# ShangtongZhang/DeepRL

Hardware: NVIDIA H100
Metric: gradient-updates/sec (DQN batch 512, 84x84x4 synthetic) (higher is better)
Workload: dtype bf16

## Files before the change

deeprl_b200/csrc/gemm.cu:

```cuda
#include <cuda.h>
#include <cstdlib>
#include "common.cuh"
#include "wgmma.cuh"

namespace b2rl {

constexpr int GEMM_BM = 128;
constexpr int GEMM_BK = 64;
constexpr int GEMM_THREADS = 384;
constexpr int MMA_WARPS = 8;

__device__ __forceinline__ uint32_t s2u(const void* p) { return (uint32_t)__cvta_generic_to_shared(p); }

__device__ __forceinline__ void mb_init(uint64_t* bar, uint32_t count) {
  asm volatile("mbarrier.init.shared::cta.b64 [%0], %1;" ::"r"(s2u(bar)), "r"(count));
}
__device__ __forceinline__ void mb_expect_tx(uint64_t* bar, uint32_t bytes) {
  asm volatile("mbarrier.arrive.expect_tx.shared::cta.b64 _, [%0], %1;" ::"r"(s2u(bar)), "r"(bytes) : "memory");
}
__device__ __forceinline__ void mb_arrive(uint64_t* bar) {
  asm volatile("mbarrier.arrive.shared::cta.b64 _, [%0];" ::"r"(s2u(bar)) : "memory");
}
__device__ __forceinline__ void mb_wait(uint64_t* bar, uint32_t parity) {
  asm volatile(
// ... 655 lines not shown
__device__ __forceinline__ uint32_t lds32(uint32_t addr) {
  uint32_t v;
  asm volatile("ld.shared.u32 %0, [%1];" : "=r"(v) : "r"(addr));
  return v;
}
__device__ __forceinline__ void sts128(uint32_t addr, const int4 v) {
  asm volatile("st.shared.v4.b32 [%0], {%1, %2, %3, %4};" ::"r"(addr), "r"(v.x), "r"(v.y), "r"(v.z), "r"(v.w) : "memory");
}

__device__ __forceinline__ uint32_t slab_chunk(uint32_t slab, uint32_t slab_b, int rl, int j) {
  return j < 8 ? slab + (uint32_t)(rl * 128 + ((j ^ (rl & 7)) << 4)) : slab_b + (uint32_t)(rl * 32 + (((j - 8) ^ ((rl >> 2) & 1)) << 4));
}

template <int J0, int NJ>
__device__ __forceinline__ void u8_store_chunks(uint32_t stage, uint32_t slab, uint32_t slab_b, int rl, int so, int fstride,
                                                int frame_w) {
  uint32_t w0[NJ], w1[NJ];
#pragma unroll
  for (int jj = 0; jj < NJ; ++jj) {
    const int j = J0 + jj;
    w0[jj] = w1[jj] = 0;
    if (so >= 0) {
      const uint32_t src = stage + (uint32_t)((j >> 1) * fstride + so + (2 * (j & 1)) * frame_w);
      w0[jj] = lds32(src);
      w1[jj] = lds32(src + frame_w);
    }
  }
#pragma unroll
  for (int jj = 0; jj < NJ; ++jj) sts128(slab_chunk(slab, slab_b, rl, J0 + jj), cvt8_u8_bf16(w0[jj], w1[jj]));
}

template <int NT, int NCH>
__device__ __forceinline__ void u8_convert(const U8Src& u, const uint8_t* stage_p, uint8_t* slab_p, uint8_t* slab_b_p, int R0,
                                           int slab_rows, int slots, int tid, int bar_id) {
  const uint32_t stage = s2u(stage_p), slab = s2u(slab_p), slab_b = NCH > 8 ? s2u(slab_b_p) : 0u;
  const int rowb = 4 * u.frame_w, fstride = slots * rowb;
  const int q0 = R0 / u.G;
  const int qb1 = (q0 / u.G + 1) * u.G;
  const int seg1 = (u.nf * fstride + 127) & ~127;
  const int rl0 = tid & 127;
  if (rl0 < slab_rows) {
    const int r = R0 + rl0;
    int so = -1;
    if (r < u.rows) {
      const int q = r / u.G;
      so = (q >= qb1 ? seg1 + (q - qb1) * rowb : (q - q0) * rowb) + 4 * (r - q * u.G);
    }
    if (NT == 128) {
      u8_store_chunks<0, NCH>(stage, slab, slab_b, rl0, so, fstride, u.frame_w);
    } else if (tid < 128) {
      u8_store_chunks<0, NCH / 2>(stage, slab, slab_b, rl0, so, fstride, u.frame_w);
    } else {
      u8_store_chunks<NCH / 2, NCH / 2>(stage, slab, slab_b, rl0, so, fstride, u.frame_w);
    }
  }
  for (int e = tid; e < (slab_rows - 128) * NCH; e += NT) {
    const int rl = 128 + e / NCH, j = e % NCH, r = R0 + rl;
    uint32_t w0 = 0, w1 = 0;
    if (r < u.rows) {
      const int q = r / u.G;
      const uint32_t src = stage + (uint32_t)((j >> 1) * fstride + (q >= qb1 ? seg1 + (q - qb1) * rowb : (q - q0) * rowb) +
                                              4 * (r - q * u.G) + (2 * (j & 1)) * u.frame_w);
      w0 = lds32(src);
      w1 = lds32(src + u.frame_w);
    }
    sts128(slab_chunk(slab, slab_b, rl, j), cvt8_u8_bf16(w0, w1));
  }
  asm volatile("fence.proxy.async.shared::cta;" ::: "memory");
  asm volatile("bar.sync %0, %1;" ::"r"(bar_id), "n"(NT) : "memory");
}

struct SlabParams {
  GemmParams g;
  int taps, col_blocks;
  int slab_rows;
  int min_shift;
  int stages;
  int base_offset_mode;
  U8Src u8;
  unsigned long long* clk;
};

enum { K1_CLK_CTA, K1_CLK_PRODUCER_WAIT, K1_CLK_CONVERT_WAIT_SLAB, K1_CLK_CONVERT_WAIT_PIXELS, K1_CLK_CONVERT, K1_CLK_MMA_WAIT,
       K1_CLK_MMA, K1_CLK_EPILOGUE, K1_CLK_EPILOGUE_STAGE, K1_CLK_TILES, K1_CLK_SLOTS };
__device__ __forceinline__ long long clk_now(const unsigned long long* clk) { return clk ? clock64() : 0; }

constexpr int SLAB_U8_THREADS = GEMM_THREADS + 128;

__host__ __device__ inline uint32_t pair_block_b_bytes(int slab_rows) { return ((uint32_t)slab_rows * 32 + 1023) & ~1023u; }
__device__ __forceinline__ uint64_t make_desc_sw32(uint32_t smem_addr) {
  return (uint64_t)((smem_addr >> 4) & 0x3FFF) | ((uint64_t)1 << 16) | ((uint64_t)(256 >> 4) << 32) | ((uint64_t)3 << 62);
}
template <int BN, bool EXT, bool U8, int TX, int TY, int CB, bool PAIR>
__device__ __forceinline__ void conv_slab_body(const CUtensorMap& tmA, const CUtensorMap& tmB, const CUtensorMap& tmA2,
                                               const CUtensorMap& tmB2, const SlabParams& sp) {
  static_assert(!PAIR || (U8 && !EXT && BN == 64 && TX == 2 && TY == 2 && CB == 1), "the paired forward is conv1's K1 shape");
  const int n_cta = sp.g.dual ? (int)(gridDim.x >> 1) : (int)gridDim.x;
  const bool second = sp.g.dual && (int)blockIdx.x >= n_cta;
  const int cta = second ? (int)blockIdx.x - n_cta : (int)blockIdx.x;
  const CUtensorMap* mA = second ? &tmA2 : &tmA;
  const CUtensorMap* mB = second ? &tmB2 : &tmB;
  GemmParams p = sp.g;
  if (second) { p.D = sp.g.D2; p.bias = sp.g.bias2; }
  constexpr uint32_t W_TILE = BN * 128;
  constexpr uint32_t WB_TILE = BN * 32;
  constexpr int ACC_LD = acc_ld(BN);
  constexpr int MAX_STAGES = 6;
  extern __shared__ __align__(1024) uint8_t smem_raw[];
  uint8_t* smem = reinterpret_cast<uint8_t*>((reinterpret_cast<uintptr_t>(smem_raw) + 1023) & ~uintptr_t(1023));
  constexpr int k_tiles = TX * TY * CB;
  const uint32_t slab_block = (uint32_t)sp.slab_rows * 128;
  const uint32_t slab_bytes = slab_block * CB + (PAIR ? pair_block_b_bytes(sp.slab_rows) : 0u);
  uint8_t* sW = smem;
  uint8_t* sWB = smem + (size_t)k_tiles * W_TILE;
  uint8_t* sS = sWB + (PAIR ? (size_t)k_tiles * WB_TILE : 0);
  float* sAcc = reinterpret_cast<float*>(sS + (size_t)sp.stages * slab_bytes);
  uint64_t* full = reinterpret_cast<uint64_t*>(sAcc + GEMM_BM * ACC_LD);
  uint64_t* empty = full + MAX_STAGES;
  uint64_t* w_full = empty + MAX_STAGES;
  const int u8_slots_ = U8 ? u8_slots(sp.slab_rows, sp.u8.G) : 0;
  const int u8_bytes = U8 ? u8_stage_bytes(sp.slab_rows, sp.u8.G, sp.u8.frame_w, sp.u8.nf) : 0;
  uint8_t* sU = reinterpret_cast<uint8_t*>((reinterpret_cast<uintptr_t>(w_full + 2) + 127) & ~uintptr_t(127));
  const int U8_STAGES = U8 ? sp.u8.stages : 1;
  uint64_t* u8_full = reinterpret_cast<uint64_t*>(sU + (size_t)U8_STAGES * u8_bytes);
  uint64_t* u8_empty = u8_full + U8_MAX_STAGES;

  const int warp = __shfl_sync(0xffffffffu, threadIdx.x >> 5, 0), lane = threadIdx.x & 31;
  const int tiles = (p.M + GEMM_BM - 1) / GEMM_BM;

  __shared__ float s_dbias[128];
  if (threadIdx.x < 128) s_dbias[threadIdx.x] = 0.0f;
  if (threadIdx.x == 0) {
    for (int s = 0; s < MAX_STAGES; ++s) { mb_init(&full[s], 1); mb_init(&empty[s], MMA_WARPS / 2); }
    mb_init(w_full, 1);
    if (U8) {
      for (int s = 0; s < U8_STAGES; ++s) { mb_init(&u8_full[s], 1); mb_init(&u8_empty[s], 1); }
    }
    asm volatile("fence.mbarrier_init.release.cluster;" ::: "memory");
    asm volatile("prefetch.tensormap [%0];" ::"l"(mA) : "memory");
    asm volatile("prefetch.tensormap [%0];" ::"l"(mB) : "memory");
    if (PAIR) {
      asm volatile("prefetch.tensormap [%0];" ::"l"(&tmA2) : "memory");
      asm volatile("prefetch.tensormap [%0];" ::"l"(&tmB2) : "memory");
    }
  }
  if constexpr (PAIR) {
    for (int i = threadIdx.x; i < k_tiles * (int)WB_TILE / 32; i += blockDim.x)
      sts128(s2u(sWB) + (uint32_t)((i / 64) * WB_TILE + (i % 64) * 16), make_int4(0, 0, 0, 0));
    asm volatile("fence.proxy.async.shared::cta;" ::: "memory");
  }
  __syncthreads();
  pdl_sync();
  unsigned long long* const clk = U8 ? sp.clk : nullptr;
  const long long t_start = clk_now(clk);
  long long c_wait = 0, c_wait2 = 0, c_work = 0, c_epi = 0, c_stage = 0;
  if (warp < 4) {
    if constexpr (!U8) asm volatile("setmaxnreg.dec.sync.aligned.u32 56;");
    if (warp == 0 && elect_one()) {
    if constexpr (PAIR) {
      mb_expect_tx(w_full, (uint32_t)k_tiles * (W_TILE + WB_TILE / 2));
      for (int kt = 0; kt < k_tiles; ++kt) {
        tma_load_3d(sW + (size_t)kt * W_TILE, mB, w_full, 0, kt, 0);
        tma_load_3d(sW + (size_t)kt * W_TILE + W_TILE / 2, &tmA2, w_full, -16, kt, 0);
        tma_load_3d(sWB + (size_t)kt * WB_TILE + WB_TILE / 2, &tmB2, w_full, 48, kt, 0);
      }
    } else {
      mb_expect_tx(w_full, (uint32_t)k_tiles * W_TILE);
      for (int kt = 0; kt < k_tiles; ++kt) tma_load_2d(sW + (size_t)kt * W_TILE, mB, w_full, kt * GEMM_BK, 0);
    }
    if constexpr (U8) {
      const int nimg = sp.u8.rows / (sp.u8.G * sp.u8.G);
      U8Plan pl = u8_plan(sp.u8, cta * GEMM_BM + sp.min_shift, sp.slab_rows);
      long long i0 = 0, i1 = 0;
      if (cta < tiles && pl.n0 > 0) { i0 = __ldg(sp.u8.idx + pl.b0); i1 = __ldg(sp.u8.idx + min(pl.b0 + 1, nimg - 1)); }
      uint32_t it = 0;
      for (int tile = cta; tile < tiles; tile += n_cta, ++it) {
        const U8Plan cur = pl;
        const long long c0 = i0, c1 = i1;
        if (tile + n_cta < tiles) {
          pl = u8_plan(sp.u8, (tile + n_cta) * GEMM_BM + sp.min_shift, sp.slab_rows);
          if (pl.n0 > 0) { i0 = __ldg(sp.u8.idx + pl.b0); i1 = __ldg(sp.u8.idx + min(pl.b0 + 1, nimg - 1)); }
        }
        const int us = it % U8_STAGES;
        const long long t0 = clk_now(clk);
        mb_wait(&u8_empty[us], ((it / U8_STAGES) & 1) ^ 1);
        c_wait += clk_now(clk) - t0;
        u8_issue(sp.u8, mA, cur, c0, c1, sU + (size_t)us * u8_bytes, &u8_full[us], u8_slots_);
      }
      if (clk) atomicAdd(clk + K1_CLK_PRODUCER_WAIT, (unsigned long long)c_wait);
    } else {
      uint32_t it = 0;
      for (int tile = cta; tile < tiles; tile += n_cta, ++it) {
        const int s = it % sp.stages;
        mb_wait(&empty[s], ((it / sp.stages) & 1) ^ 1);
        mb_expect_tx(&full[s], slab_bytes);
        for (int cb = 0; cb < CB; ++cb)
          tma_load_2d(sS + (size_t)s * slab_bytes + (size_t)cb * slab_block, mA, &full[s], cb * GEMM_BK,
                      tile * GEMM_BM + sp.min_shift);
        if (EXT && p.mask) {
          const int r0 = tile * GEMM_BM, nr = min(GEMM_BM, p.M - r0);
          prefetch_l2_bulk(p.mask + (int64_t)r0 * p.mask_ld, (uint32_t)(((int64_t)(nr - 1) * p.mask_ld + p.N) * 2));
        }
      }
    }
    }
  } else if (U8 && warp >= 12) {
    const int tid = (int)threadIdx.x - GEMM_THREADS;
    uint32_t it = 0;
    for (int tile = cta; tile < tiles; tile += n_cta, ++it) {
      const int s = it % sp.stages, us = it % U8_STAGES;
      const long long t0 = clk_now(clk);
      mb_wait(&empty[s], ((it / sp.stages) & 1) ^ 1);
      const long long t1 = clk_now(clk);
      mb_wait(&u8_full[us], (it / U8_STAGES) & 1);
      const long long t2 = clk_now(clk);
      u8_convert<128, PAIR ? 10 : 8>(sp.u8, sU + (size_t)us * u8_bytes, sS + (size_t)s * slab_bytes,
                                     sS + (size_t)s * slab_bytes + slab_block, tile * GEMM_BM + sp.min_shift, sp.slab_rows,
                                     u8_slots_, tid, 4);
      if (tid == 0) { mb_arrive(&full[s]); mb_arrive(&u8_empty[us]); }
      c_wait += t1 - t0, c_wait2 += t2 - t1, c_work += clk_now(clk) - t2;
    }
    if (clk && tid == 0) {
      atomicAdd(clk + K1_CLK_CONVERT_WAIT_SLAB, (unsigned long long)c_wait);
      atomicAdd(clk + K1_CLK_CONVERT_WAIT_PIXELS, (unsigned long long)c_wait2);
      atomicAdd(clk + K1_CLK_CONVERT, (unsigned long long)c_work);
    }
  } else {
    if constexpr (!U8) asm volatile("setmaxnreg.inc.sync.aligned.u32 224;");
    const int cw = warp - 4, g = cw >> 2, wl = cw & 3;
    const int t = wl * 32 + lane;
    float* sAcc_g = sAcc + g * 64 * ACC_LD;
    const uint32_t w0 = s2u(sW), wb0 = s2u(sWB);
    mb_wait(w_full, 0);
    uint32_t it = g;
    int n_tiles_g = 0;
    for (int tile = cta + g * n_cta; tile < tiles; tile += 2 * n_cta, it += 2) {
      const int s = it % sp.stages;
      const long long t0 = clk_now(clk);
      if (it > 0) named_sync(5 + g, 256);
      mb_wait(&full[s], (it / sp.stages) & 1);
      const long long t1 = clk_now(clk);
      float d[2][BN / 2];
      acc_zero<BN>(d[0]);
      acc_zero<BN>(d[1]);
      acc_fence<BN>(d[0]);
      acc_fence<BN>(d[1]);
      const uint32_t slab = s2u(sS) + (uint32_t)s * slab_bytes;
      wg_fence();
#pragma unroll
      for (int dy = 0; dy < TY; ++dy) {
#pragma unroll
        for (int dx = 0; dx < TX; ++dx) {
#pragma unroll
          for (int cb = 0; cb < CB; ++cb) {
            const uint64_t b = make_desc(w0 + ((dy * TX + dx) * CB + cb) * W_TILE, 16);
#pragma unroll
            for (int h = 0; h < 2; ++h) {
              const int row = 64 * h - sp.min_shift + p.shift_sign * (dy * p.grid_w + dx);
              const uint32_t a_addr = slab + cb * slab_block + (uint32_t)row * 128;
              mma_ktile<BN, 0, 0>(d[h], make_desc(a_addr, 16, sp.base_offset_mode == 1 ? (a_addr >> 7) & 7 : 0), b);
              if constexpr (PAIR)
                wgmma_n64<0, 0>(d[h], make_desc_sw32(slab + slab_block + (uint32_t)row * 32),
                                make_desc_sw32(wb0 + (dy * TX + dx) * WB_TILE));
            }
          }
        }
      }
      wg_commit();
      if (tile + n_cta < tiles) named_arrive(5 + (g ^ 1), 256);
      int4 mk[2][BN / 16];
      if constexpr (BN <= 64) epi_mask_load<BN, EXT>(p, tile * GEMM_BM, 0, t, mk[0]);
      wg_wait0();
      acc_fence<BN>(d[0]);
      acc_fence<BN>(d[1]);
      if (lane == 0) mb_arrive(&empty[s]);
      const long long t2 = clk_now(clk);
      if constexpr (BN > 64) epi_mask_load<BN, EXT>(p, tile * GEMM_BM, 0, t, mk[0]);
#pragma unroll
      for (int h = 0; h < 2; ++h) {
        if (BN > 64 && h == 1) epi_mask_load<BN, EXT>(p, tile * GEMM_BM + 64, 0, t, mk[1]);
        const long long t3 = clk_now(clk);
        stage_acc<BN>(d[h], sAcc_g, ACC_LD, wl, lane);
        named_sync(2 + g, 128);
        c_stage += clk_now(clk) - t3;
        if (BN <= 64 && h == 0) epi_mask_load<BN, EXT>(p, tile * GEMM_BM + 64, 0, t, mk[1]);
        epilogue_half<BN, EXT, PAIR>(p, tile * GEMM_BM + 64 * h, 0, t, sAcc_g, mk[h], s_dbias);
        named_sync(2 + g, 128);
      }
      c_wait += t1 - t0, c_work += t2 - t1, c_epi += clk_now(clk) - t2, ++n_tiles_g;
    }
    if (clk && t == 0) {
      atomicAdd(clk + K1_CLK_MMA_WAIT, (unsigned long long)c_wait);
      atomicAdd(clk + K1_CLK_MMA, (unsigned long long)c_work);
      atomicAdd(clk + K1_CLK_EPILOGUE, (unsigned long long)c_epi);
      atomicAdd(clk + K1_CLK_EPILOGUE_STAGE, (unsigned long long)c_stage);
      atomicAdd(clk + K1_CLK_TILES, (unsigned long long)n_tiles_g);
    }
  }
  __syncthreads();
  if (clk && threadIdx.x == 0) atomicAdd(clk + K1_CLK_CTA, (unsigned long long)(clock64() - t_start));
  if (EXT && sp.g.dbias && (int)threadIdx.x < dbias_slots(sp.g)) atomicAdd(sp.g.dbias + threadIdx.x, s_dbias[threadIdx.x]);
}

template <int BN, bool EXT, bool U8, int TX, int TY, int CB>
__global__ void __launch_bounds__(U8 ? SLAB_U8_THREADS : GEMM_THREADS, 1) conv_slab_wgmma_kernel(const __grid_constant__ CUtensorMap tmA,
                                                                          const __grid_constant__ CUtensorMap tmB,
                                                                          const __grid_constant__ CUtensorMap tmA2,
                                                                          const __grid_constant__ CUtensorMap tmB2,
                                                                          const SlabParams sp) {
  conv_slab_body<BN, EXT, U8, TX, TY, CB, false>(tmA, tmB, tmA2, tmB2, sp);
}
__global__ void __launch_bounds__(SLAB_U8_THREADS, 1) conv1_pair_wgmma_kernel(const __grid_constant__ CUtensorMap tmA,
                                                                             const __grid_constant__ CUtensorMap tmB,
                                                                             const __grid_constant__ CUtensorMap tmA2,
                                                                             const __grid_constant__ CUtensorMap tmB2,
                                                                             const SlabParams sp) {
  conv_slab_body<64, false, true, 2, 2, 1, true>(tmA, tmB, tmA2, tmB2, sp);
}


struct WgradParams {
  int rows, n_out, C, col_blocks;
  int tap0, ntaps, taps_x, grid_w;
  int slab_rows, stages, k_tiles_per_cta, a_boxes;
  float* D;
  int ldd;
  int64_t partial_stride;
  int n_runs;
  int win0;
  uint32_t run_off[9], run_acc[9];
  int stack_delta, stack_rows;
  int run_low[9];
};

constexpr int WGRAD_N128 = 0, WGRAD_2X64 = 1, WGRAD_1X64 = 2;
template <int WIN>
__global__ void __launch_bounds__(GEMM_THREADS, 1) conv_wgrad_wgmma_kernel(const __grid_constant__ CUtensorMap tmG,
                                                                          const __grid_constant__ CUtensorMap tmX,
                                                                          const WgradParams w) {
  constexpr int MAX_STAGES = 6;
  constexpr uint32_t A_BYTES = 2 * 8192;
  extern __shared__ __align__(1024) uint8_t smem_raw[];
  uint8_t* smem = reinterpret_cast<uint8_t*>((reinterpret_cast<uintptr_t>(smem_raw) + 1023) & ~uintptr_t(1023));
  const uint32_t slab_block = (uint32_t)w.slab_rows * 128, slab_bytes = slab_block * w.col_blocks;
  const uint32_t stage_bytes = A_BYTES + slab_bytes;
  uint64_t* full = reinterpret_cast<uint64_t*>(smem + (size_t)w.stages * stage_bytes);
  uint64_t* empty = full + MAX_STAGES;
  const int warp = __shfl_sync(0xffffffffu, threadIdx.x >> 5, 0), lane = threadIdx.x & 31;
  const int kt_total = (w.rows + GEMM_BK - 1) / GEMM_BK;
  const int kt_begin = blockIdx.x * w.k_tiles_per_cta;
  const int n_kt = max(min(kt_total, kt_begin + w.k_tiles_per_cta) - kt_begin, 0);

  if (threadIdx.x == 0) {
    for (int s = 0; s < MAX_STAGES; ++s) { mb_init(&full[s], 1); mb_init(&empty[s], MMA_WARPS); }
    asm volatile("fence.mbarrier_init.release.cluster;" ::: "memory");
    asm volatile("prefetch.tensormap [%0];" ::"l"(&tmG) : "memory");
    asm volatile("prefetch.tensormap [%0];" ::"l"(&tmX) : "memory");
  }
  __syncthreads();
  pdl_sync();

  if (warp == 0 && elect_one()) {
    for (int i = 0; i < n_kt; ++i) {
      const int s = i % w.stages;
      mb_wait(&empty[s], ((i / w.stages) & 1) ^ 1);
      mb_expect_tx(&full[s], (uint32_t)w.a_boxes * 8192 + slab_bytes);
      uint8_t* st = smem + (size_t)s * stage_bytes;
      const int k0 = (kt_begin + i) * GEMM_BK;
      for (int g = 0; g < w.a_boxes; ++g)
        tma_load_2d(st + g * 8192, &tmG, &full[s], w.stack_delta ? 0 : g * 64, k0 + (g ? w.stack_delta : 0));
      for (int cb = 0; cb < w.col_blocks; ++cb)
        tma_load_2d(st + A_BYTES + (size_t)cb * slab_block, &tmX, &full[s], cb * GEMM_BK, k0);
    }
  } else if (warp >= 4 && n_kt > 0 && (warp - 4) / 4 >= w.a_boxes) {
    for (int i = 0; i < n_kt; ++i) {
      mb_wait(&full[i % w.stages], (i / w.stages) & 1);
      if (lane == 0) mb_arrive(&empty[i % w.stages]);
    }
  } else if (warp >= 4 && n_kt > 0) {
    constexpr int NJ = WIN == WGRAD_2X64 ? 2 : 1, WC = WIN == WGRAD_N128 ? 128 : 64;
    const int cw = warp - 4, g = cw >> 2, wl = cw & 3;
    const int j0 = w.win0 + (int)blockIdx.y * NJ;
    const uint64_t a0 = make_desc(s2u(smem) + g * 8192, 8192);
    const uint32_t b0 = s2u(smem) + A_BYTES + w.run_off[j0] * 16;
    const uint32_t b1 = s2u(smem) + A_BYTES + w.run_off[NJ > 1 ? j0 + 1 : j0] * 16;
    float d[NJ * WC / 2];
    acc_zero<NJ * WC>(d);
    for (int i = 0; i < n_kt; ++i) {
      const int s = i % w.stages;
      mb_wait(&full[s], (i / w.stages) & 1);
      const uint32_t st = (uint32_t)s * stage_bytes;
      const uint64_t a = a0 + (st >> 4);
      wg_fence();
      if constexpr (WIN == WGRAD_N128) {
        mma_ktile<128, 1, 1>(d, a, make_desc(b0 + st, slab_block));
// ... 384 lines not shown
  cudaLaunchKernelEx(&cfg, k, ta, tb, p);
  return check_launch("b2rl_gemm_bf16");
}

template <int BN, int STAGES, bool EXT>
static int launch_dense_bn(const CUtensorMap& ta, const CUtensorMap& tb, const GemmParams& p, int splits, int cluster,
                           cudaStream_t st) {
  if constexpr (BN >= 64) {
    if (p.b_mn) {
      if (!p.a_mn) return launch_dense_t<BN, STAGES, 0, 1, EXT>(ta, tb, p, splits, cluster, st);
      if constexpr (!EXT) return launch_dense_t<BN, STAGES, 1, 1, false>(ta, tb, p, splits, cluster, st);
    }
  }
  if (!p.b_mn) {
    if (!p.a_mn) return launch_dense_t<BN, STAGES, 0, 0, EXT>(ta, tb, p, splits, cluster, st);
    if constexpr (!EXT) return launch_dense_t<BN, STAGES, 1, 0, false>(ta, tb, p, splits, cluster, st);
  }
  set_error("b2rl_gemm_bf16: no kernel for a_mn %d, b_mn %d, block_n %d%s", p.a_mn, p.b_mn, BN, EXT ? " with backward extras" : "");
  return B2RL_ERR_ARG;
}

static int dense_dispatch(const uint16_t* A, int a_mn, int64_t lda, int64_t a_rows, int64_t a_cols, const uint16_t* B,
                          int b_mn, int64_t ldb, int64_t b_rows, int64_t b_cols, GemmParams p, int splits, int block_n,
                          int cluster, cudaStream_t st) {
  CUtensorMap ta, tb;
  int rc = make_map(&ta, A, a_cols, a_rows, lda, a_mn ? 64 : GEMM_BM);
  if (rc) return rc;
  rc = make_map(&tb, B, b_cols, b_rows, ldb, b_mn ? 64 : block_n);
  if (rc) return rc;
  const int kt_total = (p.K + GEMM_BK - 1) / GEMM_BK;
  if (splits > kt_total) splits = kt_total;
  p.k_tiles_per_split = (kt_total + splits - 1) / splits;
  splits = (kt_total + p.k_tiles_per_split - 1) / p.k_tiles_per_split;
  const bool ext = has_ext(p);
  if (block_n == 32) return ext ? launch_dense_bn<32, 6, true>(ta, tb, p, splits, cluster, st)
                                : launch_dense_bn<32, 6, false>(ta, tb, p, splits, cluster, st);
  if (block_n == 64) return ext ? launch_dense_bn<64, 6, true>(ta, tb, p, splits, cluster, st)
                                : launch_dense_bn<64, 6, false>(ta, tb, p, splits, cluster, st);
  return ext ? launch_dense_bn<128, 4, true>(ta, tb, p, splits, cluster, st)
             : launch_dense_bn<128, 4, false>(ta, tb, p, splits, cluster, st);
}

template <int BN, bool EXT, bool U8, int TX, int TY, int CB, bool PAIR>
static auto slab_kernel() {
  if constexpr (PAIR) return &conv1_pair_wgmma_kernel;
  else return &conv_slab_wgmma_kernel<BN, EXT, U8, TX, TY, CB>;
}

template <int BN, bool EXT, bool U8, int TX, int TY, int CB, bool PAIR = false>
static int launch_slab_t(const CUtensorMap& ta, const CUtensorMap& tb, const CUtensorMap& ta2, const CUtensorMap& tb2,
                         SlabParams sp, cudaStream_t st) {
  const size_t w_bytes = (size_t)TX * TY * CB * BN * 128 + (PAIR ? (size_t)TX * TY * BN * 32 : 0);
  const size_t slab_bytes = (size_t)sp.slab_rows * 128 * CB + (PAIR ? pair_block_b_bytes(sp.slab_rows) : 0);
  const int tiles = (sp.g.M + GEMM_BM - 1) / GEMM_BM;
  const size_t fixed = 1024 + acc_stage_bytes(BN) + (2 * 6 + 2) * 8 + 128;
  auto k = slab_kernel<BN, EXT, U8, TX, TY, CB, PAIR>();
  static const size_t limit = dyn_smem_limit(k);
  if (limit <= fixed) return 1;
  size_t u8_extra = 0;
  size_t budget = limit - fixed;
  if (U8) {
    const size_t ub = u8_stage_bytes(sp.slab_rows, sp.u8.G, sp.u8.frame_w, sp.u8.nf);
    if (w_bytes + 3 * slab_bytes + 2 * ub + 2 * U8_MAX_STAGES * 8 > budget) return 1;
    int us = (int)((budget - w_bytes - 3 * slab_bytes - 2 * U8_MAX_STAGES * 8) / ub);
    if (us > U8_MAX_STAGES) us = U8_MAX_STAGES;
    sp.u8.stages = us;
    u8_extra = (size_t)us * ub + 2 * U8_MAX_STAGES * 8;
    budget = w_bytes + 3 * slab_bytes;
  }
  if (w_bytes + 2 * slab_bytes > budget) return 1;
  int stages = (int)((budget - w_bytes) / slab_bytes);
  if (stages > 6) stages = 6;
  sp.stages = stages;
  const size_t smem = fixed + w_bytes + stages * slab_bytes + u8_extra;
  static size_t attr = 0;
  if (attr < smem) {
    cudaFuncSetAttribute(k, cudaFuncAttributeMaxDynamicSharedMemorySize, (int)smem);
    attr = smem;
  }
  int ctas = sp.g.dual ? grid_cap() / 2 : grid_cap();
  if (ctas > tiles) ctas = tiles;
  if (ctas < 1) ctas = 1;
  g_last_ctas = sp.g.dual ? 2 * ctas : ctas;
  launch_pdl(k, dim3(sp.g.dual ? 2 * ctas : ctas), dim3(U8 ? SLAB_U8_THREADS : GEMM_THREADS), smem, st, ta, tb, ta2, tb2, sp);
  return check_launch("b2rl_conv_gemm_bf16(slab)");
}

template <int BN, bool EXT>
static int launch_slab_shape(const CUtensorMap& ta, const CUtensorMap& tb, const CUtensorMap& ta2, const CUtensorMap& tb2,
                             const SlabParams& sp, cudaStream_t st) {
  const int tx = sp.g.taps_x, ty = sp.taps / sp.g.taps_x, cb = sp.col_blocks;
  if (tx * ty != sp.taps) return 1;
  if constexpr (BN == 32) {
    if (tx == 2 && ty == 2 && cb == 1) return launch_slab_t<32, EXT, false, 2, 2, 1>(ta, tb, ta2, tb2, sp, st);
  } else if constexpr (BN == 64) {
    if (tx == 2 && ty == 2 && cb == 2) return launch_slab_t<64, EXT, false, 2, 2, 2>(ta, tb, ta2, tb2, sp, st);
    if (tx == 3 && ty == 3 && cb == 1) return launch_slab_t<64, EXT, false, 3, 3, 1>(ta, tb, ta2, tb2, sp, st);
  } else {
    if (tx == 2 && ty == 2 && cb == 1) return launch_slab_t<128, EXT, false, 2, 2, 1>(ta, tb, ta2, tb2, sp, st);
  }
  return 1;
}

template <int BN>
static int launch_slab(const CUtensorMap& ta, const CUtensorMap& tb, const CUtensorMap& ta2, const CUtensorMap& tb2,
                       SlabParams sp, cudaStream_t st) {
  if (sp.u8.frames) {
    if constexpr (BN == 32) {
      if (!has_ext(sp.g) && !sp.g.dual && sp.col_blocks == 1 && sp.taps == 4 && sp.g.taps_x == 2)
        return launch_slab_t<32, false, true, 2, 2, 1>(ta, tb, ta2, tb2, sp, st);
    }
    set_error("the uint8-ring producer serves block_n 32, 2x2 taps of 64 channels, no backward extras, no dual launch");
    return B2RL_ERR_ARG;
  }
  return has_ext(sp.g) ? launch_slab_shape<BN, true>(ta, tb, ta2, tb2, sp, st)
                       : launch_slab_shape<BN, false>(ta, tb, ta2, tb2, sp, st);
}

template <int WIN>
static void launch_wgrad_k(const CUtensorMap& tg, const CUtensorMap& tx, const WgradParams& w, int ctas, int groups,
                           size_t smem, cudaStream_t st) {
  auto k = conv_wgrad_wgmma_kernel<WIN>;
  static size_t attr = 0;
  if (attr < smem) {
    cudaFuncSetAttribute(k, cudaFuncAttributeMaxDynamicSharedMemorySize, (int)smem);
    attr = smem;
  }
  launch_pdl(k, dim3(ctas, groups), dim3(GEMM_THREADS), smem, st, tg, tx, w);
}

static int launch_wgrad(const CUtensorMap& tg, const CUtensorMap& tx, WgradParams w, cudaStream_t st, int* n_ctas = nullptr) {
  const size_t slab_bytes = (size_t)w.slab_rows * 128 * w.col_blocks, stage = 16384 + slab_bytes;
  static const size_t limit = dyn_smem_limit(conv_wgrad_wgmma_kernel<WGRAD_2X64>);
  const size_t fixed = 1024 + 2 * 6 * 8 + 16;
  const size_t budget = limit > fixed + 200 * 1024 ? 200 * 1024 : (limit > fixed ? limit - fixed : 0);
  int stages = (int)(budget / stage);
  if (stages > 6) stages = 6;
  if (stages < 2) return 1;
  w.stages = stages;
  const size_t smem = 1024 + stages * stage + 2 * 6 * 8 + 16;
  if (w.ntaps > 9 || (w.C != 64 && w.C != 128)) return 1;
  for (int n = 0; n < w.ntaps; ++n) {
    const int tap = w.tap0 + n, dy = tap / w.taps_x, dx = tap - dy * w.taps_x;
    w.run_off[n] = (uint32_t)(dy * w.grid_w + dx) * 8;
    w.run_acc[n] = (uint32_t)(n * w.C);
    w.run_low[n] = (w.stack_delta && dy == w.stack_rows - 2) ? ((dy + 1) * w.taps_x + dx) * w.C : -1;
  }
  w.n_runs = w.ntaps;
  const int groups = (w.ntaps * w.C + 127) / 128;
  const int kt_total = (w.rows + GEMM_BK - 1) / GEMM_BK;
  int ctas = kt_total / 4;
  if (ctas > grid_cap() / groups) ctas = grid_cap() / groups;
  static int cap = -1;
  if (cap < 0) {
    const char* e = getenv("B2RL_WGRAD_CTAS");
    cap = e ? atoi(e) : 0;
  }
  if (cap > 0 && ctas > cap) ctas = cap;
  if (ctas < 1) ctas = 1;
  w.k_tiles_per_cta = (kt_total + ctas - 1) / ctas;
  ctas = (kt_total + w.k_tiles_per_cta - 1) / w.k_tiles_per_cta;
  if (n_ctas) *n_ctas = ctas;
  g_last_ctas = ctas * groups;
  w.win0 = 0;
  if (w.C == 128) {
    launch_wgrad_k<WGRAD_N128>(tg, tx, w, ctas, groups, smem, st);
  } else {
// ... 61 lines not shown
  B2RL_REQUIRE(ctas >= 0, "the CTA budget is a CTA count (0: every SM)");
  g_cta_budget = ctas;
  return B2RL_OK;
}

extern "C" int b2rl_last_grid_ctas(int32_t* ctas) {
  B2RL_REQUIRE(ctas, "null pointer");
  *ctas = g_last_ctas;
  return B2RL_OK;
}

static int check_common(const void* A, const void* B, const void* D, int64_t lda, int64_t ldb, int M, int N, int K,
                        int out_mode, int splits, int block_n, int b_mn, int relu) {
  B2RL_REQUIRE(A && B && D, "null pointer");
  B2RL_REQUIRE(M > 0 && N > 0 && K > 0, "bad shape");
  B2RL_REQUIRE(lda % 8 == 0 && ldb % 8 == 0, "operand row strides must be multiples of 8 elements (16 bytes)");
  B2RL_REQUIRE((reinterpret_cast<uintptr_t>(A) | reinterpret_cast<uintptr_t>(B)) % 16 == 0, "operands must be 16-byte aligned");
  B2RL_REQUIRE(out_mode >= 0 && out_mode <= 2, "out_mode 0 (bf16) | 1 (fp32) | 2 (fp32 atomic add)");
  B2RL_REQUIRE(block_n == 32 || block_n == 64 || block_n == 128, "block_n must be 32, 64 or 128");
  B2RL_REQUIRE(!(b_mn && block_n < 64), "MN-major B needs block_n >= 64");
  B2RL_REQUIRE(splits >= 1 && (splits == 1 || out_mode == 2), "split-K needs out_mode 2 (atomic fp32 accumulation)");
  B2RL_REQUIRE(!(relu && out_mode == 2), "ReLU cannot be fused into an atomic accumulation");
  return B2RL_OK;
}

extern "C" int b2rl_gemm_bf16(const uint16_t* A, int32_t a_mn, int64_t lda, const uint16_t* B, int32_t b_mn, int64_t ldb,
                              void* D, int64_t ldd, int32_t M, int32_t N, int32_t K, const float* bias, int32_t relu,
                              int32_t out_mode, int32_t splits, int32_t block_n, void* stream) {
  int rc = check_common(A, B, D, lda, ldb, M, N, K, out_mode, splits, block_n, b_mn, relu);
  if (rc) return rc;
  GemmParams p = {};
  p.M = M; p.N = N; p.K = K; p.ldd = (int)ldd;
  p.a_mn = a_mn; p.b_mn = b_mn; p.relu = relu; p.out_mode = out_mode; p.bias = bias; p.D = D;
  p.taps_x = 1; p.shift_sign = 1;
  return dense_dispatch(A, a_mn, lda, a_mn ? K : M, a_mn ? M : K, B, b_mn, ldb, b_mn ? K : N, b_mn ? N : K, p, splits,
                        block_n, 0, (cudaStream_t)stream);
}

static int apply_ext(GemmParams& p, const b2rl_bwd_epilogue* ext, int N) {
  B2RL_REQUIRE(!ext->mask || (ext->mask_ld % 8 == 0 && reinterpret_cast<uintptr_t>(ext->mask) % 16 == 0 && N % 32 == 0),
               "mask rows must be 16-byte aligned and N a multiple of 32");
  B2RL_REQUIRE(!ext->dbias || (ext->dbias_mod >= 0 && ext->dbias_mod <= 128), "dbias_mod must be in [0, 128] (0: one bias per column)");
  B2RL_REQUIRE(p.out_map < 3 || (ext->sub_c > 0 && ext->sub_c % 32 == 0 && N % ext->sub_c == 0),
               "scatter maps need sub_c a multiple of 32 that divides N");
  p.mask = reinterpret_cast<const __nv_bfloat16*>(ext->mask);
  p.mask_ld = ext->mask_ld;
  p.dbias = ext->dbias;
  p.dbias_mod = ext->dbias ? ext->dbias_mod : 1;
  p.sub_c = ext->sub_c > 0 ? ext->sub_c : 32;
  return B2RL_OK;
}

static int conv_gemm_impl(int32_t mode, const uint16_t* X, int64_t rows, int32_t C, const uint16_t* W_or_G, int32_t n_out,
                          int32_t taps, int32_t taps_x, int32_t grid_w, int32_t shift_sign, void* D, int64_t ldd,
                          const float* bias, int32_t relu, int32_t out_mode, int32_t out_map, int32_t G, int32_t V,
                          int32_t splits, int32_t block_n, void* stream, const uint16_t* X2 = nullptr,
                          const uint16_t* W2 = nullptr, void* D2 = nullptr, const float* bias2 = nullptr,
                          const b2rl_bwd_epilogue* ext = nullptr) {
  B2RL_REQUIRE(mode == 0 || mode == 1, "mode 0 (forward/dgrad) or 1 (wgrad)");
  B2RL_REQUIRE(rows > 0 && C > 0 && taps > 0 && taps_x > 0 && n_out > 0, "bad shape");
  B2RL_REQUIRE(out_map >= 0 && out_map <= (ext ? 4 : 2), "bad out_map");
  GemmParams p = {};
  p.relu = relu; p.out_mode = out_mode; p.bias = bias; p.D = D; p.ldd = (int)ldd;
  p.taps_x = taps_x; p.grid_w = grid_w; p.shift_sign = shift_sign;
  p.out_map = out_map; p.G = G; p.V = V;
  p.dual = X2 != nullptr; p.D2 = D2; p.bias2 = bias2;
  if (ext) {
    int rc0 = apply_ext(p, ext, n_out);
    if (rc0) return rc0;
  }
  if (mode == 0) {
    B2RL_REQUIRE(C % 64 == 0, "forward/dgrad needs channels in multiples of 64");
    const int K = taps * C;
    int rc = check_common(X, W_or_G, D, C, K, (int)rows, n_out, K, out_mode, splits, block_n, 0, relu);
    if (rc) return rc;
    p.M = (int)rows; p.N = n_out; p.K = K; p.a_mn = 0; p.b_mn = 0; p.a_tap_tiles = C / 64;
    if (g_use_slab && splits == 1 && n_out <= block_n && out_mode != 2) {
      const int max_shift = ((taps - 1) / taps_x) * grid_w + (taps - 1) % taps_x;
      SlabParams sp = {};
      sp.g = p; sp.taps = taps; sp.col_blocks = C / 64;
      sp.slab_rows = (GEMM_BM + max_shift + 7) / 8 * 8;
      sp.min_shift = shift_sign > 0 ? 0 : -max_shift;
      sp.base_offset_mode = g_use_slab;
      if (sp.slab_rows <= 256) {
        CUtensorMap ta, tb, ta2, tb2;
        rc = make_map(&ta, X, C, rows, C, sp.slab_rows);
        if (rc) return rc;
        rc = make_map(&tb, W_or_G, K, n_out, K, block_n);
        if (rc) return rc;
        ta2 = ta, tb2 = tb;
        if (p.dual) {
          rc = make_map(&ta2, X2, C, rows, C, sp.slab_rows);
          if (rc) return rc;
          rc = make_map(&tb2, W2, K, n_out, K, block_n);
          if (rc) return rc;
        }
        int r2 = block_n == 32 ? launch_slab<32>(ta, tb, ta2, tb2, sp, (cudaStream_t)stream)
                 : block_n == 64 ? launch_slab<64>(ta, tb, ta2, tb2, sp, (cudaStream_t)stream)
                                 : launch_slab<128>(ta, tb, ta2, tb2, sp, (cudaStream_t)stream);
        if (r2 <= 0) return r2;
      }
    }
    return gemm_dispatch(X, 0, C, rows, C, W_or_G, 0, K, n_out, K, p, splits, block_n, (cudaStream_t)stream, X2, W2);
  }
  B2RL_REQUIRE(!p.dual, "the dual launch is for forward / dgrad GEMMs");
  B2RL_REQUIRE(C % block_n == 0, "wgrad needs channels in multiples of block_n");
  B2RL_REQUIRE(n_out % 8 == 0, "wgrad needs n_out in multiples of 8");
  int rc = check_common(W_or_G, X, D, n_out, C, n_out, taps * C, (int)rows, out_mode, splits, block_n, 1, relu);
  if (rc) return rc;
  B2RL_REQUIRE(out_mode == 2, "wgrad accumulates with out_mode 2");
  if (g_use_slab && C % 64 == 0 && C <= 128 && n_out <= 128 && shift_sign > 0 && ldd % 2 == 0 &&
      reinterpret_cast<uintptr_t>(g_wgrad_partials ? g_partial_buf : D) % 8 == 0) {
    int max_shift = ((taps - 1) / taps_x) * grid_w + (taps - 1) % taps_x;
    WgradParams w = {};
    w.rows = (int)rows; w.n_out = n_out; w.C = C; w.col_blocks = C / 64; w.taps_x = taps_x; w.grid_w = grid_w;
    w.a_boxes = n_out > 64 ? 2 : 1;
    static int stack_on = -1;
    if (stack_on < 0) {
      const char* e = getenv("B2RL_WGRAD_STACK");
      stack_on = (e && atoi(e) == 0) ? 0 : 1;
    }
    const int taps_y = taps / taps_x;
    int win_taps = taps;
    if (stack_on && n_out <= 64 && taps_y >= 2 && taps_y * taps_x == taps) {
      w.stack_delta = -grid_w; w.stack_rows = taps_y; w.a_boxes = 2;
      win_taps = (taps_y - 1) * taps_x;
      max_shift = (taps_y - 2) * grid_w + taps_x - 1;
    }
    w.slab_rows = (GEMM_BK + max_shift + 7) / 8 * 8;
    w.D = reinterpret_cast<float*>(D); w.ldd = (int)ldd;
    if (g_wgrad_partials) { w.D = g_partial_buf; w.partial_stride = g_partial_stride; }
    CUtensorMap tg, tx;
    rc = make_map(&tg, W_or_G, n_out, rows, n_out, 64);
    if (rc) return rc;
    rc = make_map(&tx, X, C, rows, C, w.slab_rows);
    if (rc) return rc;
    w.tap0 = 0;
    w.ntaps = win_taps;
    const int r2 = launch_wgrad(tg, tx, w, (cudaStream_t)stream, &g_partial_count);
    if (r2 <= 0) return r2;
  }
  p.M = n_out; p.N = taps * C; p.K = (int)rows; p.a_mn = 1; p.b_mn = 1; p.b_tap_tiles = C / block_n;
  return gemm_dispatch(W_or_G, 1, n_out, rows, n_out, X, 1, C, rows, C, p, splits, block_n, (cudaStream_t)stream);
}

extern "C" int b2rl_conv_gemm_bf16(int32_t mode, const uint16_t* X, int64_t rows, int32_t C, const uint16_t* W_or_G,
                                   int32_t n_out, int32_t taps, int32_t taps_x, int32_t grid_w, int32_t shift_sign,
                                   void* D, int64_t ldd, const float* bias, int32_t relu, int32_t out_mode,
                                   int32_t out_map, int32_t G, int32_t V, int32_t splits, int32_t block_n, void* stream) {
  return conv_gemm_impl(mode, X, rows, C, W_or_G, n_out, taps, taps_x, grid_w, shift_sign, D, ldd, bias, relu, out_mode,
                        out_map, G, V, splits, block_n, stream);
}

extern "C" int b2rl_conv_gemm_dual_bf16(const uint16_t* X, const uint16_t* X2, int64_t rows, int32_t C, const uint16_t* W,
                                        const uint16_t* W2, int32_t n_out, int32_t taps, int32_t taps_x, int32_t grid_w,
                                        int32_t shift_sign, void* D, void* D2, int64_t ldd, const float* bias,
                                        const float* bias2, int32_t relu, int32_t out_mode, int32_t out_map, int32_t G,
                                        int32_t V, int32_t block_n, void* stream) {
  B2RL_REQUIRE(X2 && W2 && D2, "null pointer in the second operand set");
  B2RL_REQUIRE((reinterpret_cast<uintptr_t>(X2) | reinterpret_cast<uintptr_t>(W2)) % 16 == 0, "operands must be 16-byte aligned");
  B2RL_REQUIRE((bias == nullptr) == (bias2 == nullptr), "both or neither bias");
  return conv_gemm_impl(0, X, rows, C, W, n_out, taps, taps_x, grid_w, shift_sign, D, ldd, bias, relu, out_mode, out_map, G,
                        V, 1, block_n, stream, X2, W2, D2, bias2);
}

extern "C" int b2rl_gemm_dual_bf16(const uint16_t* A, const uint16_t* A2, int64_t lda, const uint16_t* B, const uint16_t* B2,
// ... 253 lines not shown
```

Before: 3519.

## Split slab conv kernel into dedicated MMA and epilogue warpgroups

Restructures the slab conv kernel from two MMA warpgroups that each ran their own epilogue into one MMA warpgroup plus two epilogue warpgroups, each handling one 64-row half. The MMA warpgroup stages accumulators to shared memory and hands off through named barriers, so the epilogue overlaps the next tile's MMA. Per-role register budgets are set with setmaxnreg and the block grows to 512/640 threads. Clock instrumentation is extended to the non-u8 path. The single MMA warpgroup may now be the bottleneck, and the extra barrier handoffs add synchronisation cost.

```diff
diff --git a/deeprl_b200/csrc/gemm.cu b/deeprl_b200/csrc/gemm.cu
--- a/deeprl_b200/csrc/gemm.cu
+++ b/deeprl_b200/csrc/gemm.cu
@@ -761,10 +761,18 @@
 };
 
 enum { K1_CLK_CTA, K1_CLK_PRODUCER_WAIT, K1_CLK_CONVERT_WAIT_SLAB, K1_CLK_CONVERT_WAIT_PIXELS, K1_CLK_CONVERT, K1_CLK_MMA_WAIT,
-       K1_CLK_MMA, K1_CLK_EPILOGUE, K1_CLK_EPILOGUE_STAGE, K1_CLK_TILES, K1_CLK_SLOTS };
+       K1_CLK_MMA, K1_CLK_MMA_WAIT_FREE, K1_CLK_MMA_STAGE, K1_CLK_EPILOGUE_WAIT, K1_CLK_EPILOGUE, K1_CLK_TILES, K1_CLK_SLOTS };
 __device__ __forceinline__ long long clk_now(const unsigned long long* clk) { return clk ? clock64() : 0; }
 
 constexpr int SLAB_U8_THREADS = GEMM_THREADS + 128;
+constexpr int SLAB_THREADS = 512;
+constexpr int SLAB_K1_THREADS = SLAB_THREADS + 128;
+constexpr int SLAB_BAR_STAGED = 5, SLAB_BAR_FREE = 7;
+template <bool U8> struct SlabRegs;
+template <> struct SlabRegs<false> { static constexpr int producer = 40, mma = 232, epilogue = 120, convert = 0; };
+template <> struct SlabRegs<true> { static constexpr int producer = 64, mma = 136, epilogue = 88, convert = 104; };
+template <int R> __device__ __forceinline__ void reg_dec() { asm volatile("setmaxnreg.dec.sync.aligned.u32 %0;" ::"n"(R)); }
+template <int R> __device__ __forceinline__ void reg_inc() { asm volatile("setmaxnreg.inc.sync.aligned.u32 %0;" ::"n"(R)); }
 
 __host__ __device__ inline uint32_t pair_block_b_bytes(int slab_rows) { return ((uint32_t)slab_rows * 32 + 1023) & ~1023u; }
 __device__ __forceinline__ uint64_t make_desc_sw32(uint32_t smem_addr) {
@@ -830,11 +838,15 @@
   }
   __syncthreads();
   pdl_sync();
-  unsigned long long* const clk = U8 ? sp.clk : nullptr;
+  unsigned long long* const clk = sp.clk;
   const long long t_start = clk_now(clk);
-  long long c_wait = 0, c_wait2 = 0, c_work = 0, c_epi = 0, c_stage = 0;
+  long long c_wait = 0, c_wait2 = 0, c_work = 0, c_stage = 0;
+  using R = SlabRegs<U8>;
+  constexpr int launch_regs = 65536 / (U8 ? SLAB_K1_THREADS : SLAB_THREADS) / 8 * 8;
+  static_assert(R::producer + R::mma + 2 * R::epilogue + R::convert <= (U8 ? 5 : 4) * launch_regs,
+                "the roles' register shares exceed what the launch allocates");
   if (warp < 4) {
-    if constexpr (!U8) asm volatile("setmaxnreg.dec.sync.aligned.u32 56;");
+    reg_dec<R::producer>();
     if (warp == 0 && elect_one()) {
     if constexpr (PAIR) {
       mb_expect_tx(w_full, (uint32_t)k_tiles * (W_TILE + WB_TILE / 2));
@@ -871,7 +883,9 @@
       uint32_t it = 0;
       for (int tile = cta; tile < tiles; tile += n_cta, ++it) {
         const int s = it % sp.stages;
+        const long long t0 = clk_now(clk);
         mb_wait(&empty[s], ((it / sp.stages) & 1) ^ 1);
+        c_wait += clk_now(clk) - t0;
         mb_expect_tx(&full[s], slab_bytes);
         for (int cb = 0; cb < CB; ++cb)
           tma_load_2d(sS + (size_t)s * slab_bytes + (size_t)cb * slab_block, mA, &full[s], cb * GEMM_BK,
@@ -881,10 +895,12 @@
           prefetch_l2_bulk(p.mask + (int64_t)r0 * p.mask_ld, (uint32_t)(((int64_t)(nr - 1) * p.mask_ld + p.N) * 2));
         }
       }
-    }
-    }
-  } else if (U8 && warp >= 12) {
-    const int tid = (int)threadIdx.x - GEMM_THREADS;
+      if (clk) atomicAdd(clk + K1_CLK_PRODUCER_WAIT, (unsigned long long)c_wait);
+    }
+    }
+  } else if (U8 && warp >= 16) {
+    reg_inc<R::convert>();
+    const int tid = (int)threadIdx.x - SLAB_THREADS;
     uint32_t it = 0;
     for (int tile = cta; tile < tiles; tile += n_cta, ++it) {
       const int s = it % sp.stages, us = it % U8_STAGES;
@@ -904,19 +920,16 @@
       atomicAdd(clk + K1_CLK_CONVERT_WAIT_PIXELS, (unsigned long long)c_wait2);
       atomicAdd(clk + K1_CLK_CONVERT, (unsigned long long)c_work);
     }
-  } else {
-    if constexpr (!U8) asm volatile("setmaxnreg.inc.sync.aligned.u32 224;");
-    const int cw = warp - 4, g = cw >> 2, wl = cw & 3;
-    const int t = wl * 32 + lane;
-    float* sAcc_g = sAcc + g * 64 * ACC_LD;
+  } else if (warp < 8) {
+    reg_inc<R::mma>();
+    const int wl = warp - 4;
     const uint32_t w0 = s2u(sW), wb0 = s2u(sWB);
     mb_wait(w_full, 0);
-    uint32_t it = g;
-    int n_tiles_g = 0;
-    for (int tile = cta + g * n_cta; tile < tiles; tile += 2 * n_cta, it += 2) {
+    long long c_free = 0;
+    uint32_t it = 0;
+    for (int tile = cta; tile < tiles; tile += n_cta, ++it) {
       const int s = it % sp.stages;
       const long long t0 = clk_now(clk);
-      if (it > 0) named_sync(5 + g, 256);
       mb_wait(&full[s], (it / sp.stages) & 1);
       const long long t1 = clk_now(clk);
       float d[2][BN / 2];
@@ -946,34 +959,47 @@
         }
       }
       wg_commit();
-      if (tile + n_cta < tiles) named_arrive(5 + (g ^ 1), 256);
-      int4 mk[2][BN / 16];
-      if constexpr (BN <= 64) epi_mask_load<BN, EXT>(p, tile * GEMM_BM, 0, t, mk[0]);
       wg_wait0();
       acc_fence<BN>(d[0]);
       acc_fence<BN>(d[1]);
       if (lane == 0) mb_arrive(&empty[s]);
       const long long t2 = clk_now(clk);
-      if constexpr (BN > 64) epi_mask_load<BN, EXT>(p, tile * GEMM_BM, 0, t, mk[0]);
 #pragma unroll
       for (int h = 0; h < 2; ++h) {
-        if (BN > 64 && h == 1) epi_mask_load<BN, EXT>(p, tile * GEMM_BM + 64, 0, t, mk[1]);
         const long long t3 = clk_now(clk);
-        stage_acc<BN>(d[h], sAcc_g, ACC_LD, wl, lane);
-        named_sync(2 + g, 128);
-        c_stage += clk_now(clk) - t3;
-        if (BN <= 64 && h == 0) epi_mask_load<BN, EXT>(p, tile * GEMM_BM + 64, 0, t, mk[1]);
-        epilogue_half<BN, EXT, PAIR>(p, tile * GEMM_BM + 64 * h, 0, t, sAcc_g, mk[h], s_dbias);
-        named_sync(2 + g, 128);
-      }
-      c_wait += t1 - t0, c_work += t2 - t1, c_epi += clk_now(clk) - t2, ++n_tiles_g;
-    }
-    if (clk && t == 0) {
+        if (it > 0) named_sync(SLAB_BAR_FREE + h, 256);
+        const long long t4 = clk_now(clk);
+        stage_acc<BN>(d[h], sAcc + h * 64 * ACC_LD, ACC_LD, wl, lane);
+        named_arrive(SLAB_BAR_STAGED + h, 256);
+        c_free += t4 - t3, c_stage += clk_now(clk) - t4;
+      }
+      c_wait += t1 - t0, c_work += t2 - t1;
+    }
+    if (clk && wl == 0 && lane == 0) {
       atomicAdd(clk + K1_CLK_MMA_WAIT, (unsigned long long)c_wait);
       atomicAdd(clk + K1_CLK_MMA, (unsigned long long)c_work);
-      atomicAdd(clk + K1_CLK_EPILOGUE, (unsigned long long)c_epi);
-      atomicAdd(clk + K1_CLK_EPILOGUE_STAGE, (unsigned long long)c_stage);
-      atomicAdd(clk + K1_CLK_TILES, (unsigned long long)n_tiles_g);
+      atomicAdd(clk + K1_CLK_MMA_WAIT_FREE, (unsigned long long)c_free);
+      atomicAdd(clk + K1_CLK_MMA_STAGE, (unsigned long long)c_stage);
+      atomicAdd(clk + K1_CLK_TILES, (unsigned long long)it);
+    }
+  } else {
+    reg_dec<R::epilogue>();
+    const int e = (warp - 8) >> 2, wl = (warp - 8) & 3;
+    const int t = wl * 32 + lane;
+    const float* sAcc_e = sAcc + e * 64 * ACC_LD;
+    for (int tile = cta; tile < tiles; tile += n_cta) {
+      int4 mk[BN / 16];
+      epi_mask_load<BN, EXT>(p, tile * GEMM_BM + 64 * e, 0, t, mk);
+      const long long t0 = clk_now(clk);
+      named_sync(SLAB_BAR_STAGED + e, 256);
+      const long long t1 = clk_now(clk);
+      epilogue_half<BN, EXT, PAIR>(p, tile * GEMM_BM + 64 * e, 0, t, sAcc_e, mk, s_dbias);
+      if (tile + n_cta < tiles) named_arrive(SLAB_BAR_FREE + e, 256);
+      c_wait += t1 - t0, c_work += clk_now(clk) - t1;
+    }
+    if (clk && t == 0) {
+      atomicAdd(clk + K1_CLK_EPILOGUE_WAIT, (unsigned long long)c_wait);
+      atomicAdd(clk + K1_CLK_EPILOGUE, (unsigned long long)c_work);
     }
   }
   __syncthreads();
@@ -982,14 +1008,14 @@
 }
 
 template <int BN, bool EXT, bool U8, int TX, int TY, int CB>
-__global__ void __launch_bounds__(U8 ? SLAB_U8_THREADS : GEMM_THREADS, 1) conv_slab_wgmma_kernel(const __grid_constant__ CUtensorMap tmA,
+__global__ void __launch_bounds__(U8 ? SLAB_K1_THREADS : SLAB_THREADS, 1) conv_slab_wgmma_kernel(const __grid_constant__ CUtensorMap tmA,
                                                                           const __grid_constant__ CUtensorMap tmB,
                                                                           const __grid_constant__ CUtensorMap tmA2,
                                                                           const __grid_constant__ CUtensorMap tmB2,
                                                                           const SlabParams sp) {
   conv_slab_body<BN, EXT, U8, TX, TY, CB, false>(tmA, tmB, tmA2, tmB2, sp);
 }
-__global__ void __launch_bounds__(SLAB_U8_THREADS, 1) conv1_pair_wgmma_kernel(const __grid_constant__ CUtensorMap tmA,
+__global__ void __launch_bounds__(SLAB_K1_THREADS, 1) conv1_pair_wgmma_kernel(const __grid_constant__ CUtensorMap tmA,
                                                                              const __grid_constant__ CUtensorMap tmB,
                                                                              const __grid_constant__ CUtensorMap tmA2,
                                                                              const __grid_constant__ CUtensorMap tmB2,
@@ -1540,7 +1566,7 @@
   if (ctas > tiles) ctas = tiles;
   if (ctas < 1) ctas = 1;
   g_last_ctas = sp.g.dual ? 2 * ctas : ctas;
-  launch_pdl(k, dim3(sp.g.dual ? 2 * ctas : ctas), dim3(U8 ? SLAB_U8_THREADS : GEMM_THREADS), smem, st, ta, tb, ta2, tb2, sp);
+  launch_pdl(k, dim3(sp.g.dual ? 2 * ctas : ctas), dim3(U8 ? SLAB_K1_THREADS : SLAB_THREADS), smem, st, ta, tb, ta2, tb2, sp);
   return check_launch("b2rl_conv_gemm_bf16(slab)");
 }
 
@@ -1768,6 +1794,7 @@
       sp.slab_rows = (GEMM_BM + max_shift + 7) / 8 * 8;
       sp.min_shift = shift_sign > 0 ? 0 : -max_shift;
       sp.base_offset_mode = g_use_slab;
+      sp.clk = g_k1_clocks;
       if (sp.slab_rows <= 256) {
         CUtensorMap ta, tb, ta2, tb2;
         rc = make_map(&ta, X, C, rows, C, sp.slab_rows);
```

Result: faster. 3752 (median of 6 runs) (+6.6%).
